# openai/multiagent-particle-envs

Measured on AMD Instinct MI355X. Metric: env steps/sec (whole node), simple_spread N=3, batch=65536 per GPU, higher is better.
Workload: dtype f32; 1 GPU; simple_spread A=3 L=3, 65536 worlds/GPU, fresh one-hot moves, reset every 25 steps; steps commanded to the step server; protocol=fresh, step-server (one doorbell per episode), batch_per_gpu=65536, global_batch=65536, mode=step-server, commands=auto, barrier_backend=none

## Files before the change

multiagent_particle_envs_amd/csrc/mpe_split.hip:

```cpp
#include <type_traits>

#include "mpe_internal.h"

#ifndef MPE_SPLIT_ABLATE
#define MPE_SPLIT_ABLATE 0
#endif

#ifdef MPE_PHASE_CLOCK
#define MPE_STAMP(k)                                                                                              \
  do {                                                                                                            \
    if (blockIdx.x < 4 && lane == 0 && b.force && t < 32)                                                         \
      reinterpret_cast<unsigned long long *>(b.force)[(((size_t)blockIdx.x * 16 + role) * 32 + t) * 8 + (k)] =     \
          __builtin_amdgcn_s_memtime();                                                                           \
  } while (0)
#else
#define MPE_STAMP(k) do { } while (0)
#endif

#ifdef MPE_DEVICE_SPAN
#define MPE_SPAN_BEGIN() const unsigned long long span_t0_ = (unsigned long long)wall_clock64()
#define MPE_SPAN_END()                                                                                             \
  do {                                                                                                             \
    if (b_in.force && (threadIdx.x & 63) == 0 && (threadIdx.x >> 6) < 8) {                                           \
      const uintptr_t sp_ = reinterpret_cast<uintptr_t>(b_in.force);                                                \
// ... 302 lines not shown
    for (int g = 0; g < NG; ++g)
#pragma unroll
      for (int v = 0; v < NADV; ++v) {
        const float d2 = sq2d(px[NADV + g] - px[v], py[NADV + g] - py[v]);
        hit[g][v] = sqrt_lt(d2, sz[NADV + g] + sz[v]);
        dmin[v] = fminf(dmin[v], d2);
      }
    float fx[2], fy[2];
#pragma unroll
    for (int f = 0; f < 2; ++f) {
      fx[f] = ROLL ? food_roll[2 * f] : (b.pos + wave_off((size_t)(2 * (A + 1 + f)) * B + w0))[ln];
      fy[f] = ROLL ? food_roll[2 * f + 1] : (b.pos + wave_off((size_t)(2 * (A + 1 + f) + 1) * B + w0))[ln];
    }
    if (live) {
#pragma unroll
      for (int a = 0; a < A; ++a) {
        float r = 0.f;
        if (a < NADV) {
          r = r - 0.1f * fast_sqrt(dmin[a < NADV ? a : 0]);
          if ((d.collide >> a) & 1u) {
#pragma unroll
            for (int g = 0; g < NG; ++g)
#pragma unroll
              for (int v = 0; v < NADV; ++v) r = r + (hit[g][v] ? 5.f : 0.f);
          }
        } else {
          if ((d.collide >> a) & 1u) {
#pragma unroll
            for (int v = 0; v < NADV; ++v) r = r - (hit[a >= NADV ? a - NADV : 0][v] ? 5.f : 0.f);
          }
          r = r - 2.f * tag_bound(fabsf(px[a]));
          r = r - 2.f * tag_bound(fabsf(py[a]));
          float m2 = INFINITY;
#pragma unroll
          for (int f = 0; f < 2; ++f) {
            const float d2 = sq2d(px[a] - fx[f], py[a] - fy[f]);
            r = r + (sqrt_lt(d2, sz[a] + sz[A + 1 + f]) ? 2.f : 0.f);
            m2 = fminf(m2, d2);
          }
          r = r + 0.05f * fast_sqrt(m2);
        }
        const size_t o = ro + (size_t)a * B;
        if (b.rew) store_aux<AUX>(b.rew + wave_off(o) + ln, r);
        if (b.done) store_aux<AUX>(b.done + wave_off(o) + ln, 0);
        if (b.info_collisions) {
          int c = 0;
          if (a < NADV) {
#pragma unroll
            for (int g = 0; g < NG; ++g) c += hit[g][a < NADV ? a : 0] ? 1 : 0;
          }
          store_aux<AUX>(b.info_collisions + wave_off(o) + ln, c);
        }
      }
    }
  }
}

typedef float vf2 __attribute__((ext_vector_type(2)));
typedef __attribute__((address_space(4))) const vf2 cvf2;
__device__ __forceinline__ vf2 pol_act2(vf2 x, bool tnh) { return vf2{pol_act(x.x, tnh), pol_act(x.y, tnh)}; }
template <int NO2>
__device__ __forceinline__ void pol_layer0(const cvf2 *W, const float *row, int sw, int D, float *rec, vf2 (&h)[NO2]) {
#pragma unroll
  for (int j = 0; j < NO2; ++j) h[j] = W[D * NO2 + j];
  for (int k = 0; k < D; ++k) {
    const float x = row[(((k >> 2) ^ sw) << 2) | (k & 3)];
    if (rec) rec[k] = x;
    const vf2 xx = {x, x};
#pragma unroll
    for (int j = 0; j < NO2; ++j) h[j] = __builtin_elementwise_fma(W[k * NO2 + j], xx, h[j]);
  }
}
template <int NO2>
__device__ __forceinline__ void pol_layer(const cvf2 *W, const vf2 (&h)[32], vf2 (&o)[NO2]) {
#pragma unroll
  for (int j = 0; j < NO2; ++j) o[j] = W[64 * NO2 + j];
#pragma unroll
  for (int k = 0; k < 64; ++k) {
    const float x = (k & 1) ? h[k >> 1].y : h[k >> 1].x;
    const vf2 xx = {x, x};
#pragma unroll
    for (int j = 0; j < NO2; ++j) o[j] = __builtin_elementwise_fma(W[k * NO2 + j], xx, o[j]);
    if ((k & 3) == 3) __builtin_amdgcn_sched_barrier(0);
  }
}
__device__ __forceinline__ void pol_logits(const float *Wg, int nl, bool tnh, const float *row, int sw, int D, float *rec,
                                           float (&z)[5]) {
  const cvf2 *W = (const cvf2 *)(uintptr_t)Wg;
  vf2 o[4];
  if (nl == 1) {
    pol_layer0<4>(W, row, sw, D, rec, o);
  } else {
    vf2 h[32];
    pol_layer0<32>(W, row, sw, D, rec, h);
#pragma unroll
    for (int j = 0; j < 32; ++j) h[j] = pol_act2(h[j], tnh);
    const cvf2 *W1 = W + (size_t)(D + 1) * 32;
    if (nl == 2) {
      pol_layer<4>(W1, h, o);
    } else {
      const cvf2 *W2 = W1 + 65 * 32;
#pragma unroll
      for (int j = 0; j < 4; ++j) o[j] = W2[64 * 4 + j];
#pragma unroll 1
      for (int c = 0; c < 4; ++c) {
        vf2 g[8];
#pragma unroll
        for (int j = 0; j < 8; ++j) g[j] = W1[64 * 32 + 8 * c + j];
#pragma unroll
        for (int k = 0; k < 64; ++k) {
          const float x = (k & 1) ? h[k >> 1].y : h[k >> 1].x;
          const vf2 xx = {x, x};
#pragma unroll
          for (int j = 0; j < 8; ++j) g[j] = __builtin_elementwise_fma(W1[k * 32 + 8 * c + j], xx, g[j]);
          if ((k & 7) == 7) __builtin_amdgcn_sched_barrier(0);
        }
#pragma unroll
        for (int u = 0; u < 16; ++u) {
          const float x = pol_act((u & 1) ? g[u >> 1].y : g[u >> 1].x, tnh);
          const vf2 xx = {x, x};
#pragma unroll
          for (int j = 0; j < 4; ++j) o[j] = __builtin_elementwise_fma(W2[(16 * c + u) * 4 + j], xx, o[j]);
        }
      }
    }
  }
  z[0] = o[0].x; z[1] = o[0].y; z[2] = o[1].x; z[3] = o[1].y; z[4] = o[2].x;
}

template <int AUX>
__device__ __forceinline__ void store_state(const MpeBuffers &b, size_t B, int i, size_t w0, unsigned ln, float mx,
                                            float my, float mvx, float mvy) {
  store_aux<AUX>(b.pos + wave_off((size_t)(2 * i) * B + w0) + ln, mx);
  store_aux<AUX>(b.pos + wave_off((size_t)(2 * i + 1) * B + w0) + ln, my);
  store_aux<AUX>(b.vel + wave_off((size_t)(2 * i) * B + w0) + ln, mvx);
  store_aux<AUX>(b.vel + wave_off((size_t)(2 * i + 1) * B + w0) + ln, mvy);
}

struct ServeArgs {
  unsigned long long *door;
  unsigned long long *flag;
  unsigned int *status;
  const float *act_ring;
  const float *comm_ring;
  int32_t ring, slots;
  unsigned long long timeout_ticks;
};
__device__ __forceinline__ unsigned long long door_load(const unsigned long long *p) {
  const unsigned long long v = __hip_atomic_load(p, __ATOMIC_RELAXED, __HIP_MEMORY_SCOPE_SYSTEM);
  const uint32_t lo = __builtin_amdgcn_readfirstlane((uint32_t)v), hi = __builtin_amdgcn_readfirstlane((uint32_t)(v >> 32));
  return ((unsigned long long)hi << 32) | lo;
}
__device__ __forceinline__ void drain_stores() { asm volatile("s_waitcnt vmcnt(0)" ::: "memory"); }

template <int KIND, int A, int L, int NADV, bool ROLL, int RP ,
          bool DUALP = false ,
          bool SERVE = false ,
          bool POL = false >
__device__ __forceinline__ void split_body(float *const g_pos, float *const g_vel, const float *const g_act, const int32_t *const g_ids,
                                           const size_t B, const int g_wpw, const int g_observe_only, const unsigned g_movable,
                                           const NarrowDesc &d, const MpeBuffers &b_in, const RollArgs &ra, const ServeArgs &sv,
                                           const PolArgs &pol) {
  static_assert(!SERVE || (ROLL && RP == kRowsSc1), "the step server: a rollout instantiation, write-through stores");
  static_assert(!POL || (ROLL && !SERVE && !DUALP), "the policy rollout: a single-role rollout instantiation");
  static_assert(!POL || KIND == MPE_SCN_SIMPLE || KIND == MPE_SCN_SPREAD || KIND == MPE_SCN_ADVERSARY || KIND == MPE_SCN_PUSH,
                "the policy rollout: scenarios whose observation rows read no other agent's velocity");
  constexpr int WM = SERVE ? kWordRowSys : (ROLL ? kWordDrawn : kWordRow);
  using S = SplitShape<KIND, A, L, NADV>;
  MPE_SPAN_BEGIN();
  MpeBuffers b = b_in;
  b.pos = g_pos;
  b.vel = g_vel;
  b.act = g_act;
  b.ids = g_ids;
  constexpr int E = A + L, XW = S::XW;
  constexpr int AUX = SERVE ? kRowsSc1 : aux_policy<KIND, RP>();
  extern __shared__ __attribute__((aligned(16))) float smem[];
  const int lane = threadIdx.x & (kWave - 1);
  constexpr bool DUAL = DUALP && ROLL;
  constexpr bool OWN_DRAW = DUAL && dual_own_draw<KIND>();
  constexpr int NAW = DUAL ? 2 * A : A;
  const int role = __builtin_amdgcn_readfirstlane((int)(threadIdx.x >> 6));
  const bool is_agent = role < NAW;
  const bool is_rows = DUAL && role >= A && role < NAW;
  const int i = is_agent ? (role >= A ? role - A : role) : 0;
  const int wpw = g_wpw;
  const size_t w0 = (size_t)blockIdx.x * (size_t)wpw;
  if (w0 >= B) return;
#ifdef MPE_STRESS_DELAY_WAVE
  if (role == (MPE_STRESS_DELAY_WAVE) % A)
    for (int k = 0; k < 10; ++k) __builtin_amdgcn_s_sleep(127);
#endif
  const int nvalid = (B - w0) < (size_t)wpw ? (int)(B - w0) : wpw;
  const bool live = lane < nvalid;
  const unsigned ln = (unsigned)(live ? lane : nvalid - 1) & 63u;
  const size_t w = w0 + (size_t)ln;
  float *const xch = smem;
  float *const tile = smem + (ROLL ? 2 : 1) * A * XW * kWave + i * S::tile_floats(ROLL);
  int *const mv = reinterpret_cast<int *>(smem + (ROLL ? 2 : 1) * A * XW * kWave + A * S::tile_floats(ROLL));

  const int T = ROLL ? ra.T : 1;
  const size_t obs_stride = (ra.trajectory || SERVE) ? (size_t)d.obs_off[A] * B : 0;
  const size_t row_stride = (ra.trajectory || SERVE) ? (size_t)A * B : 0;
  int blk0 = 0, mvt0 = 0;
  unsigned long long seen = 0;
  int *const idle_cnt = reinterpret_cast<int *>(smem + SplitShape<KIND, A, L, NADV>::lds_bytes(true) / sizeof(float));
  if constexpr (SERVE) {
    blk0 = (int)(ra.step0 % (uint64_t)sv.slots);
    mvt0 = (int)(ra.step0 % (uint64_t)sv.ring);
    if (threadIdx.x < 3) idle_cnt[threadIdx.x] = 0;
    __syncthreads();
  }
  auto block_of = [&](const int t) { return SERVE ? (blk0 + t) % sv.slots : t; };
  auto with_words = [&](const int t) {
    MpeBuffers q = b;
    if constexpr (SERVE)
      q.comm = sv.comm_ring ? sv.comm_ring + (size_t)((mvt0 + t) % sv.ring) * ((size_t)A * B * SplitShape<KIND, A, L, NADV>::DC) : nullptr;
    return q;
  };
  auto wait_door = [&](const int t, const bool publisher) -> bool {
    if constexpr (!SERVE) return true;
    const unsigned long long g = ra.step0 + (unsigned long long)t;
    if (seen > g) return true;
    seen = door_load(sv.door);
    if (seen > g) return true;
    drain_stores();
    bool told = t == 0;
    if (!publisher && !told && lane == 0) __hip_atomic_fetch_add(&idle_cnt[t & 1], 1, __ATOMIC_RELEASE, __HIP_MEMORY_SCOPE_WORKGROUP);
    const unsigned long long t_begin = (unsigned long long)wall_clock64();
    for (;;) {
      if (publisher && !told) {
        const int n = __builtin_amdgcn_readfirstlane(__hip_atomic_load(&idle_cnt[t & 1], __ATOMIC_ACQUIRE, __HIP_MEMORY_SCOPE_WORKGROUP));
        if (n >= NAW) {
          if (lane == 0) __hip_atomic_store(sv.flag + blockIdx.x, g, __ATOMIC_RELAXED, __HIP_MEMORY_SCOPE_SYSTEM);
          told = true;
        }
      }
      __builtin_amdgcn_s_sleep(4);
      seen = door_load(sv.door);
      if (seen > g) return true;
      if ((unsigned long long)wall_clock64() - t_begin > sv.timeout_ticks) {
        if (lane == 0) {
          __hip_atomic_store(sv.status, 1u, __ATOMIC_RELAXED, __HIP_MEMORY_SCOPE_SYSTEM);
          __hip_atomic_store(&idle_cnt[2], 1, __ATOMIC_RELAXED, __HIP_MEMORY_SCOPE_WORKGROUP);
        }
        return false;
      }
    }
  };
  auto next_commanded = [&](const int t) -> bool {
    if constexpr (!SERVE) return false;
    return t + 1 < T && seen > ra.step0 + (unsigned long long)t + 1;
  };
  auto aborted = [&]() -> bool {
    if constexpr (!SERVE) return false;
    return __builtin_amdgcn_readfirstlane(__hip_atomic_load(&idle_cnt[2], __ATOMIC_RELAXED, __HIP_MEMORY_SCOPE_WORKGROUP)) != 0;
  };

  if (!is_agent) {
    constexpr bool TRACK = ROLL && (KIND == MPE_SCN_CRYPTO || KIND == MPE_SCN_WORLD_COMM);
    const uint64_t gw_r = ra.world_offset + w;
    int goal_r = (ROLL && KIND == MPE_SCN_CRYPTO) ? (b.choice + wave_off(w0))[ln] : 0;
    float food[4] = {0.f, 0.f, 0.f, 0.f};
    if (ROLL && KIND == MPE_SCN_WORLD_COMM) {
#pragma unroll
      for (int f = 0; f < 2; ++f) {
        food[2 * f] = (b.pos + wave_off((size_t)(2 * (A + 1 + f)) * B + w0))[ln];
        food[2 * f + 1] = (b.pos + wave_off((size_t)(2 * (A + 1 + f) + 1) * B + w0))[ln];
      }
    }
    float sz[E];
#pragma unroll
    for (int e = 0; e < E; ++e) sz[e] = d.size[e];
    pin_s(sz);
    int cd = -1;
    uint64_t ep_r = 0;
    if (TRACK && ra.episode_len > 0) {
      const uint64_t len = (uint64_t)ra.episode_len, r = ra.step0 % len;
      cd = r == 0 ? 0 : (int)(len - r);
      ep_r = ra.step0 / len + (r ? 1 : 0);
    }
    for (int t = 0; t < T; ++t) {
      MPE_STAMP(0);
      if (SERVE && !wait_door(t, true)) {
        __syncthreads();
        return;
      }
      if (TRACK && cd >= 0) {
        if (cd == 0) {
          if (KIND == MPE_SCN_CRYPTO) goal_r = choice_draw(ra.seed, gw_r, ep_r, 0, d.choice_pop[0]);
          if (KIND == MPE_SCN_WORLD_COMM) {
#pragma unroll
            for (int f = 0; f < 2; ++f) reset_draw(ra.seed, gw_r, ep_r, A + 1 + f, ra.landmark_range, food[2 * f], food[2 * f + 1]);
          }
          ++ep_r;
          cd = ra.episode_len - 1;
        } else {
          --cd;
        }
      }
      if (ROLL && !SERVE && !OWN_DRAW && !POL && t + 1 < T) {
        const uint64_t gt1 = ra.step0 + (uint64_t)t + 1;
#pragma unroll
        for (int q = 0; q < (A + 3) / 4; ++q) {
          const U4 o = action_block(ra.seed, gw_r, gt1, q);
          const uint32_t word[4] = {o.x, o.y, o.z, o.w};
#pragma unroll
          for (int k = 0; k < 4; ++k)
            if (4 * q + k < A) mv[(((t + 1) & 1) * A + 4 * q + k) * kWave + lane] = move_of(word[k]);
        }
      }
      const float *const X = xch + (ROLL ? (t & 1) * A * XW * kWave : 0);
      MPE_STAMP(1);
      if (SERVE) drain_stores();
      __syncthreads();
      if (SERVE) {
        if (t > 0 && lane == 0) __hip_atomic_store(sv.flag + blockIdx.x, ra.step0 + (unsigned long long)t, __ATOMIC_RELAXED, __HIP_MEMORY_SCOPE_SYSTEM);
        if (lane == 0) idle_cnt[t & 1] = 0;
        if (aborted()) return;
      }
      MPE_STAMP(2);
      if (!(MPE_SPLIT_ABLATE & 2))
      reward_wave<KIND, A, L, NADV, ROLL, AUX, WM>(d, sz, with_words(t), X, lane, live, ln, B, w0, (size_t)block_of(t) * row_stride + w0,
                                                   ra.seed, gw_r, ra.step0 + (uint64_t)t, goal_r, food);
      MPE_STAMP(3);
    }
    if (SERVE) {
      drain_stores();
      __syncthreads();
      if (lane == 0) __hip_atomic_store(sv.flag + blockIdx.x, ra.step0 + (unsigned long long)T, __ATOMIC_RELAXED, __HIP_MEMORY_SCOPE_SYSTEM);
    }
    MPE_SPAN_END();
    return;
  }

  float px[E], py[E];
#pragma unroll
  for (int e = 0; e < E; ++e) {
    px[e] = (b.pos + wave_off((size_t)(2 * e) * B + w0))[ln];
    py[e] = (b.pos + wave_off((size_t)(2 * e + 1) * B + w0))[ln];
  }
  float mvx = (b.vel + wave_off((size_t)(2 * i) * B + w0))[ln];
  float mvy = (b.vel + wave_off((size_t)(2 * i + 1) * B + w0))[ln];
  const bool movable_i = (g_movable >> i) & 1u;
  const bool step_world = ROLL || !g_observe_only;
  float ux0 = 0.f, uy0 = 0.f;
  if (!ROLL && step_world && movable_i && (b.act || b.ids)) fetch_action_wave(b, B, i, w0, ln, 1.0f, ux0, uy0);

  float kc[9 + E];
  kc[0] = d.size[i]; kc[1] = d.inv_mass[i]; kc[2] = d.accel[i]; kc[3] = d.max_speed[i];
  kc[4] = d.dt; kc[5] = d.damp; kc[6] = d.cforce; kc[7] = d.cmargin; kc[8] = d.cmargin_inv;
#pragma unroll
  for (int e = 0; e < E; ++e) kc[9 + e] = d.size[e];
  pin_s(kc);
  const float size_i = kc[0], mass_i = kc[1], accel_i = kc[2], maxspd_i = kc[3];
  const float k_dt = kc[4], k_damp = kc[5], k_cforce = kc[6], k_cmargin = kc[7], k_cmargin_inv = kc[8];
  const float *const size_e = kc + 9;
  const int obs_off_i = d.obs_off[i];
  const bool collide_i = (d.collide >> i) & 1u;
  float mx = 0.f, my = 0.f;
#pragma unroll
  for (int a = 0; a < A; ++a)
    if (a == i) { mx = px[a]; my = py[a]; }

  const uint64_t gw = ra.world_offset + w;
  constexpr bool HAS_GOAL = KIND == MPE_SCN_ADVERSARY || KIND == MPE_SCN_PUSH;
  constexpr int NCH = S::NCH, DC = S::DC;
  int goal = NCH >= 1 ? (b.choice + wave_off(w0))[ln] : 0;
  int pick1 = NCH >= 2 ? (b.choice + wave_off(B + w0))[ln] : 0;

  int countdown = -1;
  uint64_t ep = 0;
  if (ROLL && ra.episode_len > 0) {
    const uint64_t len = (uint64_t)ra.episode_len, r = ra.step0 % len;
    countdown = r == 0 ? 0 : (int)(len - r);
    ep = ra.step0 / len + (r ? 1 : 0);
  }

  float gx = 0.f, gy = 0.f;
  [[maybe_unused]] bool did_reset = false;
  auto roll_reset = [&]() -> bool {
    const bool reset_now = countdown == 0;
    if (countdown >= 0) countdown = reset_now ? ra.episode_len - 1 : countdown - 1;
    if (reset_now) {
#pragma unroll
      for (int e = 0; e < E; ++e) reset_draw(ra.seed, gw, ep, e, e < A ? 1.0f : ra.landmark_range, px[e], py[e]);
#pragma unroll
      for (int a = 0; a < A; ++a)
        if (a == i) { mx = px[a]; my = py[a]; }
      mvx = 0.f;
      mvy = 0.f;
      if (NCH >= 1) goal = choice_draw(ra.seed, gw, ep, 0, d.choice_pop[0]);
      if (NCH >= 2) pick1 = choice_draw(ra.seed, gw, ep, 1, d.choice_pop[1]);
      ++ep;
      if (SERVE) did_reset = true;
    }
    return reset_now;
  };
  [[maybe_unused]] float pa1 = 0.f, pa2 = 0.f, pa3 = 0.f, pa4 = 0.f;
  auto step_forces = [&](const int t, float &fx, float &fy) {
    float ux, uy;
    const uint64_t gt = ra.step0 + (uint64_t)t;
    if (ROLL) {
      if constexpr (!POL) roll_reset();
      if constexpr (SERVE) {
        const float *const mt = sv.act_ring + (size_t)((mvt0 + t) % sv.ring) * ((size_t)A * B * MPE_ACTION_DIM);
        typedef float vf4 __attribute__((ext_vector_type(4)));
        const float *const mp = mt + wave_off(((size_t)i * B + w0) * MPE_ACTION_DIM) + (ln * MPE_ACTION_DIM + 1);
        vf4 m4;
        asm volatile("global_load_dwordx4 %0, %1, off sc0 sc1\n\ts_waitcnt vmcnt(0)" : "=&v"(m4) : "v"(mp) : "memory");
        if (movable_i) {
          ux = (m4.x - m4.y) * accel_i;
          uy = (m4.z - m4.w) * accel_i;
        } else {
          ux = 0.f;
          uy = 0.f;
        }
      } else if constexpr (POL) {
        ux = (pa1 - pa2) * accel_i;
        uy = (pa3 - pa4) * accel_i;
      } else {
      const int m = (t == 0 || OWN_DRAW) ? action_draw(ra.seed, gw, gt, i) : mv[((t & 1) * A + i) * kWave + lane];
      ux = ((m == 1 ? 1.f : 0.f) - (m == 2 ? 1.f : 0.f)) * accel_i;
      uy = ((m == 3 ? 1.f : 0.f) - (m == 4 ? 1.f : 0.f)) * accel_i;
      }
    } else if (step_world && movable_i) {
      if (b.act || b.ids) { ux = ux0 * accel_i; uy = uy0 * accel_i; }
      else fetch_action_wave(b, B, i, w0, ln, accel_i, ux, uy);
    } else {
      ux = 0.f;
      uy = 0.f;
    }
    fx = ux + 0.f;
    fy = uy + 0.f;
    if (movable_i && step_world && collide_i && !(MPE_SPLIT_ABLATE & 1)) {
#pragma unroll
      for (int j = 0; j < E; ++j) {
        if (j == i) continue;
        if (!((d.collide >> j) & 1u)) continue;
        float cx, cy;
        contact_force(mx - px[j], my - py[j], size_i + size_e[j], k_cforce, k_cmargin, k_cmargin_inv, cx, cy);
        fx = cx + fx;
        fy = cy + fy;
      }
    }
  };
  auto step_integrate = [&](const int t, const float fx, const float fy) {
    if (movable_i && step_world) {
      integrate_one(mx, my, mvx, mvy, fx, fy, mass_i, maxspd_i, k_damp, k_dt);
#ifdef MPE_STRESS_STORE_BEFORE_BARRIER
      if (live && (!ROLL || t == T - 1)) store_state<AUX>(b, B, i, w0, ln, mx, my, mvx, mvy);
#endif
    }
#ifdef MPE_PHASE_CLOCK
    asm volatile("" ::"v"(mx), "v"(my), "v"(mvx), "v"(mvy));
#endif
  };
  auto publish = [&](const int t) {
    float *const X = xch + (ROLL ? (t & 1) * A * XW * kWave : 0);
    X[(i * XW + 0) * kWave + lane] = mx;
    X[(i * XW + 1) * kWave + lane] = my;
    X[(i * XW + 2) * kWave + lane] = mvx;
    X[(i * XW + 3) * kWave + lane] = mvy;
    if (KIND == MPE_SCN_SPREAD) {
#pragma unroll
      for (int l = 0; l < L; ++l) X[(i * XW + 4 + l) * kWave + lane] = sq2d(mx - px[A + l], my - py[A + l]);
    }
    if (KIND == MPE_SCN_SIMPLE) X[(i * XW + 4) * kWave + lane] = sq2d(mx - px[A], my - py[A]);
    if (HAS_GOAL || KIND == MPE_SCN_SPEAKER_LISTENER) {
      goal_pos<A, L>(px, py, goal, gx, gy);
      X[(i * XW + 4) * kWave + lane] = sq2d(mx - gx, my - gy);
    }
    if constexpr (KIND == MPE_SCN_REFERENCE) {
      goal_pos<A, L>(px, py, i == 0 ? pick1 : goal, gx, gy);
      X[(i * XW + 4) * kWave + lane] = sq2d(mx - gx, my - gy);
    }
    if constexpr (KIND == MPE_SCN_WORLD_COMM) {
#pragma unroll
      for (int f = 0; f < 2; ++f)
        X[(i * XW + 4 + f) * kWave + lane] =
            sqrt_lt(sq2d(mx - px[A + 3 + f], my - py[A + 3 + f]), size_i + size_e[A + 3 + f]) ? 1.f : -1.f;
    }
  };
  auto behind_barrier = [&](const int t) {
#ifndef MPE_STRESS_STORE_BEFORE_BARRIER
    if (movable_i && step_world && live && (!ROLL || (SERVE ? !next_commanded(t) : t == T - 1)) && !(MPE_SPLIT_ABLATE & 8))
      store_state<AUX>(b, B, i, w0, ln, mx, my, mvx, mvy);
#endif
    if constexpr (SERVE) {
      if (did_reset && live) {
#pragma unroll
        for (int l = 0; l < L; ++l)
          if (l % A == i) {
            store_aux<AUX>(b.pos + wave_off((size_t)(2 * (A + l)) * B + w0) + ln, px[A + l]);
            store_aux<AUX>(b.pos + wave_off((size_t)(2 * (A + l) + 1) * B + w0) + ln, py[A + l]);
          }
        if (NCH >= 1 && i == 0) {
          store_aux<AUX>(b.choice + wave_off(w0) + ln, goal);
          if (NCH >= 2) store_aux<AUX>(b.choice + wave_off(B + w0) + ln, pick1);
        }
        if (!movable_i) store_state<AUX>(b, B, i, w0, ln, mx, my, mvx, mvy);
      }
      did_reset = false;
    }
    if constexpr (KIND == MPE_SCN_ADVERSARY && !ROLL) {
      if (live && b.info_rew) {
        store_aux<AUX>(b.info_rew + wave_off((size_t)i * B + w0) + ln, sq2d(mx - gx, my - gy));
        if (b.info_min_dists) {
#pragma unroll
          for (int l = 0; l < L; ++l)
            store_aux<AUX>(b.info_min_dists + wave_off(((size_t)l * A + i) * B + w0) + ln, sq2d(mx - px[A + l], my - py[A + l]));
        }
      }
    }
    const float *const X = xch + (ROLL ? (t & 1) * A * XW * kWave : 0);
#pragma unroll
    for (int a = 0; a < A; ++a) {
      if (a == i) { px[a] = mx; py[a] = my; continue; }
      px[a] = X[(a * XW + 0) * kWave + lane];
      py[a] = X[(a * XW + 1) * kWave + lane];
    }
#ifdef MPE_PHASE_CLOCK
#pragma unroll
    for (int a = 0; a < A; ++a) asm volatile("" ::"v"(px[a]), "v"(py[a]));
#endif
  };
  [[maybe_unused]] int pol_D = 0, pol_S = 0, pol_sw = 0;
  auto note_tile = [&](auto dc, auto pc) {
    if constexpr (POL) {
      constexpr int D = decltype(dc)::value;
      constexpr bool P = decltype(pc)::value;
      constexpr int NS = (P && row_vec4<D>()) ? D / 4 : 0;
      pol_D = D;
      pol_S = P ? pair_stride<D>() : tile_stride<D>();
      pol_sw = NS ? swz4<NS>(lane) : 0;
    }
  };
  auto rows = [&](const int t, const bool pre) {
    if (MPE_SPLIT_ABLATE & 4) return;
    const float *const X = xch + (ROLL ? (t & 1) * A * XW * kWave : 0);
    const uint64_t gt = ra.step0 + (uint64_t)t;
    float *const obs_t = b.obs + (size_t)block_of(t) * obs_stride;
    [[maybe_unused]] const MpeBuffers bw = with_words(t);
    if (KIND == MPE_SCN_SIMPLE) {
      constexpr int D = 2 + 2 * L;
      {
        RowPairs<D> r(tile, lane);
        r.put(0, mvx, mvy);
#pragma unroll
        for (int l = 0; l < L; ++l) r.put(2 + 2 * l, px[A + l] - mx, py[A + l] - my);
      }
      note_tile(std::integral_constant<int, D>{}, std::bool_constant<true>{});
        if (!pre) flush_rows<D, true, RP>(tile, obs_t + B * obs_off_i + w0 * D, nvalid, lane, d.vec4);
    }
    if (KIND == MPE_SCN_SPREAD) {
      constexpr int D = 4 + 2 * L + 4 * (A - 1);
      {
        RowPairs<D> r(tile, lane);
        r.put(0, mvx, mvy);
        r.put(2, mx, my);
#pragma unroll
        for (int l = 0; l < L; ++l) r.put(4 + 2 * l, px[A + l] - mx, py[A + l] - my);
        int k = 4 + 2 * L;
#pragma unroll
        for (int j = 0; j < A; ++j) {
          if (j == i) continue;
// ... 128 lines not shown
      constexpr int D = 2 + 2 * L + 3 + DC, RS = tile_stride<D>();
      const int mine = i == 0 ? goal : pick1;
      put1<RS>(tile, lane, 0, mvx); put1<RS>(tile, lane, 1, mvy);
#pragma unroll
      for (int l = 0; l < L; ++l) { put1<RS>(tile, lane, 2 + 2 * l, px[A + l] - mx); put1<RS>(tile, lane, 3 + 2 * l, py[A + l] - my); }
#pragma unroll
      for (int c = 0; c < 3; ++c) put1<RS>(tile, lane, 2 + 2 * L + c, mine == c ? 0.75f : 0.25f);
      const Word<WM> co = word_of<DC, WM>(bw, B, w0, ln, 1 - i, ra.seed, gw, gt);
#pragma unroll
      for (int c = 0; c < DC; ++c) put1<RS>(tile, lane, 5 + 2 * L + c, co[c]);
      note_tile(std::integral_constant<int, D>{}, std::bool_constant<false>{});
        if (!pre) flush_rows<D, false, RP>(tile, obs_t + B * obs_off_i + w0 * D, nvalid, lane, d.vec4);
    }
    if constexpr (KIND == MPE_SCN_CRYPTO) {
      const Word<WM> cs = word_of<DC, WM>(bw, B, w0, ln, 2, ra.seed, gw, gt);
      static_assert((DC & 1) == 0, "crypto rows are written as pairs");
      if (i == 0) {
        constexpr int D = DC;
        RowPairs<D> r(tile, lane);
#pragma unroll
        for (int c = 0; c < DC; c += 2) r.put(c, cs[c], cs[c + 1]);
        note_tile(std::integral_constant<int, D>{}, std::bool_constant<true>{});
        if (!pre) flush_rows<D, true, RP>(tile, obs_t + B * obs_off_i + w0 * D, nvalid, lane, d.vec4);
      } else {
        constexpr int D = 2 * DC;
        RowPairs<D> r(tile, lane);
        const int first = i == 1 ? pick1 : goal;
#pragma unroll
        for (int c = 0; c < DC; c += 2) r.put(c, first == c ? 1.f : 0.f, first == c + 1 ? 1.f : 0.f);
#pragma unroll
        for (int c = 0; c < DC; c += 2) {
          if (i == 1) r.put(DC + c, cs[c], cs[c + 1]);
          else        r.put(DC + c, pick1 == c ? 1.f : 0.f, pick1 == c + 1 ? 1.f : 0.f);
        }
        note_tile(std::integral_constant<int, D>{}, std::bool_constant<true>{});
        if (!pre) flush_rows<D, true, RP>(tile, obs_t + B * obs_off_i + w0 * D, nvalid, lane, d.vec4);
      }
    }
    if constexpr (KIND == MPE_SCN_WORLD_COMM) {
      constexpr int NG = A - NADV;
      constexpr int DA = 4 + 2 * L + 2 * (A - 1) + 2 * NG + 2 + DC, DGd = 4 + 2 * L + 2 * (A - 1) + 2 + 2 * (NG - 1);
      const bool f1 = X[(i * XW + 4) * kWave + lane] > 0.f, f2 = X[(i * XW + 5) * kWave + lane] > 0.f;
      bool vis[A];
#pragma unroll
      for (int j = 0; j < A; ++j) {
        const bool o1 = X[(j * XW + 4) * kWave + lane] > 0.f, o2 = X[(j * XW + 5) * kWave + lane] > 0.f;
        vis[j] = i == 0 || (f1 && o1) || (f2 && o2) || (!f1 && !o1 && !f2 && !o2);
      }
      auto row = [&](auto dsel, auto advt) {
        constexpr int D = decltype(dsel)::value, RS = tile_stride<D>();
        constexpr bool ADV = decltype(advt)::value;
        constexpr bool HALF = S::trows(ROLL) == 32;
#pragma unroll
        for (int h = 0; h < (HALF ? 2 : 1); ++h) {
        const int r = HALF ? (lane & 31) : lane;
        if (!HALF || (lane >> 5) == h) {
        int k = 0;
        put1<RS>(tile, r, 0, mvx); put1<RS>(tile, r, 1, mvy); put1<RS>(tile, r, 2, mx); put1<RS>(tile, r, 3, my);
        k = 4;
#pragma unroll
        for (int l = 0; l < L; ++l) { put1<RS>(tile, r, k, px[A + l] - mx); put1<RS>(tile, r, k + 1, py[A + l] - my); k += 2; }
#pragma unroll
        for (int j = 0; j < A; ++j) {
          if (j == i) continue;
          put1<RS>(tile, r, k, vis[j] ? px[j] - mx : 0.f);
          put1<RS>(tile, r, k + 1, vis[j] ? py[j] - my : 0.f);
          k += 2;
        }
        if (!ADV) { put1<RS>(tile, r, k, f1 ? 1.f : -1.f); put1<RS>(tile, r, k + 1, f2 ? 1.f : -1.f); k += 2; }
#pragma unroll
        for (int j = NADV; j < A; ++j) {
          if (j == i) continue;
          put1<RS>(tile, r, k, vis[j] ? X[(j * XW + 2) * kWave + lane] : 0.f);
          put1<RS>(tile, r, k + 1, vis[j] ? X[(j * XW + 3) * kWave + lane] : 0.f);
          k += 2;
        }
        if (ADV) {
          put1<RS>(tile, r, k, f1 ? 1.f : -1.f); put1<RS>(tile, r, k + 1, f2 ? 1.f : -1.f); k += 2;
          const Word<WM> cl = word_of<DC, WM>(bw, B, w0, ln, 0, ra.seed, gw, gt);
#pragma unroll
          for (int c = 0; c < DC; ++c) put1<RS>(tile, r, k + c, cl[c]);
        }
        }
        const int nv = HALF ? min(max(nvalid - 32 * h, 0), 32) : nvalid;
        if (nv > 0) flush_rows<D, false, RP>(tile, obs_t + B * obs_off_i + (w0 + (HALF ? 32 * h : 0)) * D, nv, lane, d.vec4);
        }
      };
      if (i < NADV) row(std::integral_constant<int, DA>{}, std::true_type{});
      else          row(std::integral_constant<int, DGd>{}, std::false_type{});
    }
  };
  [[maybe_unused]] auto decide = [&](const int t) {
    const uint64_t gt = ra.step0 + (uint64_t)t;
    const bool rs = roll_reset();
    if (t == 0 || rs) {
      if (HAS_GOAL) goal_pos<A, L>(px, py, goal, gx, gy);
      rows(t, true);
    }
    float *const rec = (pol.obs_in && live) ? pol.obs_in + wave_off((size_t)t * (size_t)d.obs_off[A] * B + B * (size_t)obs_off_i + w0 * (size_t)pol_D) +
                                                  ln * pol_D
                                            : nullptr;
    float z[5];
    pol_logits(pol.w + pol.off[i], pol.nl[i], pol.act[i] != 0, tile + lane * pol_S, pol_sw, pol_D, rec, z);
    float zm = z[0];
    int am = 0;
#pragma unroll
    for (int j = 1; j < 5; ++j)
      if (z[j] > zm) { zm = z[j]; am = j; }
    float e[5], sum = 0.f;
#pragma unroll
    for (int j = 0; j < 5; ++j) {
      e[j] = __expf(z[j] - zm);
      sum += e[j];
    }
    float r[5];
    int m = am;
    if (pol.mode == MPE_POLICY_SOFTMAX) {
#pragma unroll
      for (int j = 0; j < 5; ++j) r[j] = e[j] / sum;
    } else {
      if (pol.mode == MPE_POLICY_SAMPLE) {
        const float u = (float)(policy_bits(pol.seed, gw, gt, i) >> 8) * (1.0f / 16777216.0f);
        float c = 0.f;
        m = 4;
        float cj[4];
#pragma unroll
        for (int j = 0; j < 4; ++j) {
          c += e[j] / sum;
          cj[j] = c;
        }
#pragma unroll
        for (int j = 3; j >= 0; --j)
          if (u < cj[j]) m = j;
      }
#pragma unroll
      for (int j = 0; j < 5; ++j) r[j] = j == m ? 1.f : 0.f;
    }
    if (live) {
      float *const ar = pol.act_out + wave_off((((size_t)t * A + i) * B + w0) * MPE_ACTION_DIM) + ln * MPE_ACTION_DIM;
#pragma unroll
      for (int j = 0; j < 5; ++j) ar[j] = r[j];
      if (pol.logp) {
        float zsel = z[0];
#pragma unroll
        for (int j = 1; j < 5; ++j) zsel = m == j ? z[j] : zsel;
        (pol.logp + wave_off(((size_t)t * A + i) * B + w0))[ln] = (zsel - zm) - __logf(sum);
      }
    }
    pa1 = r[1];
    pa2 = r[2];
    pa3 = r[3];
    pa4 = r[4];
  };
  if constexpr (DUAL) {
    if (is_rows) {
      for (int t = 0; t < T; ++t) {
        MPE_STAMP(0);
        const bool reset_now = countdown == 0;
        if (countdown >= 0) countdown = reset_now ? ra.episode_len - 1 : countdown - 1;
        if (reset_now) {
#pragma unroll
          for (int l = 0; l < L; ++l) reset_draw(ra.seed, gw, ep, A + l, ra.landmark_range, px[A + l], py[A + l]);
          if (NCH >= 1) goal = choice_draw(ra.seed, gw, ep, 0, d.choice_pop[0]);
          if (NCH >= 2) pick1 = choice_draw(ra.seed, gw, ep, 1, d.choice_pop[1]);
          ++ep;
        }
        if (HAS_GOAL || KIND == MPE_SCN_SPEAKER_LISTENER) goal_pos<A, L>(px, py, goal, gx, gy);
        MPE_STAMP(2);
        __syncthreads();
        if (SERVE && aborted()) return;
        MPE_STAMP(3);
        const float *const X = xch + (t & 1) * A * XW * kWave;
        mx = X[(i * XW + 0) * kWave + lane];
        my = X[(i * XW + 1) * kWave + lane];
        mvx = X[(i * XW + 2) * kWave + lane];
        mvy = X[(i * XW + 3) * kWave + lane];
#pragma unroll
        for (int a = 0; a < A; ++a) {
          if (a == i) { px[a] = mx; py[a] = my; continue; }
          px[a] = X[(a * XW + 0) * kWave + lane];
          py[a] = X[(a * XW + 1) * kWave + lane];
        }
#ifdef MPE_PHASE_CLOCK
#pragma unroll
        for (int a = 0; a < A; ++a) asm volatile("" ::"v"(px[a]), "v"(py[a]));
#endif
        MPE_STAMP(4);
        rows(t, false);
        MPE_STAMP(5);
        if constexpr (SERVE) {
          drain_stores();
          if (lane == 0) __hip_atomic_fetch_add(&idle_cnt[(t + 1) & 1], 1, __ATOMIC_RELEASE, __HIP_MEMORY_SCOPE_WORKGROUP);
        }
      }
      if (SERVE) __syncthreads();
      MPE_SPAN_END();
      return;
    }
    float fx, fy;
    { [[maybe_unused]] const int t = 0; MPE_STAMP(0); }
    if (SERVE && !wait_door(0, false)) {
      __syncthreads();
      return;
    }
    step_forces(0, fx, fy);
    step_integrate(0, fx, fy);
    { [[maybe_unused]] const int t = 0; MPE_STAMP(1); }
    publish(0);
    for (int t = 0; t < T; ++t) {
      MPE_STAMP(2);
      if (SERVE) drain_stores();
      __syncthreads();
      if (SERVE && aborted()) return;
      MPE_STAMP(3);
      behind_barrier(t);
      MPE_STAMP(4);
      if (t + 1 < T) {
        if (SERVE && !wait_door(t + 1, false)) {
          __syncthreads();
          return;
        }
        step_forces(t + 1, fx, fy);
        step_integrate(t + 1, fx, fy);
        MPE_STAMP(5);
        publish(t + 1);
      }
    }
    if (SERVE) {
      drain_stores();
      __syncthreads();
      MPE_SPAN_END();
      return;
    }
  } else {
    for (int t = 0; t < T; ++t) {
      float fx, fy;
      MPE_STAMP(0);
      if (SERVE && !wait_door(t, false)) {
        __syncthreads();
        return;
      }
      if constexpr (POL) decide(t);
      step_forces(t, fx, fy);
      step_integrate(t, fx, fy);
      MPE_STAMP(1);
      publish(t);
      MPE_STAMP(2);
      if (SERVE) drain_stores();
      __syncthreads();
      if (SERVE && aborted()) return;
      MPE_STAMP(3);
      behind_barrier(t);
      MPE_STAMP(4);
      rows(t, false);
      MPE_STAMP(5);
    }
    if (SERVE) {
      drain_stores();
      __syncthreads();
      MPE_SPAN_END();
      return;
    }
  }
  if (ROLL && NCH >= 1 && ra.episode_len > 0 && live && i == 0) {
    store_aux<AUX>(b.choice + wave_off(w0) + ln, goal);
    if (NCH >= 2) store_aux<AUX>(b.choice + wave_off(B + w0) + ln, pick1);
  }
  if (ROLL && ((speakers_of<KIND>() >> i) & 1u) && live && T > 0) {
    float *const mine = const_cast<float *>(b.comm) + wave_off(((size_t)i * B + w0) * DC) + ln * DC;
    const int id = comm_draw(ra.seed, gw, ra.step0 + (uint64_t)(T - 1), i, DC);
#pragma unroll
    for (int c = 0; c < DC; ++c) mine[c] = c == id ? 1.f : 0.f;
  }
  if (ROLL && ra.episode_len > 0 && live) {
#pragma unroll
    for (int l = 0; l < L; ++l)
      if (l % A == i) {
        (b.pos + wave_off((size_t)(2 * (A + l)) * B + w0))[ln] = px[A + l];
        (b.pos + wave_off((size_t)(2 * (A + l) + 1) * B + w0))[ln] = py[A + l];
      }
    if (!movable_i) {
      store_aux<AUX>(b.pos + wave_off((size_t)(2 * i) * B + w0) + ln, mx);
      store_aux<AUX>(b.pos + wave_off((size_t)(2 * i + 1) * B + w0) + ln, my);
      store_aux<AUX>(b.vel + wave_off((size_t)(2 * i) * B + w0) + ln, mvx);
      store_aux<AUX>(b.vel + wave_off((size_t)(2 * i + 1) * B + w0) + ln, mvy);
    }
  }
  MPE_SPAN_END();
}

template <int KIND, int A, int L, int NADV, bool ROLL, int RP, bool DUALP = false, bool SERVE = false>
__global__ void __launch_bounds__((SplitShape<KIND, A, L, NADV>::waves(DUALP) * kWave))
k_split(float *const g_pos, float *const g_vel, const float *const g_act, const int32_t *const g_ids, const size_t B,
        const int g_wpw, const int g_observe_only, const unsigned g_movable, const NarrowDesc d, const MpeBuffers b_in,
        const RollArgs ra, const ServeArgs sv) {
  split_body<KIND, A, L, NADV, ROLL, RP, DUALP, SERVE, false>(g_pos, g_vel, g_act, g_ids, B, g_wpw, g_observe_only, g_movable, d, b_in,
                                                              ra, sv, PolArgs{});
}
template <int KIND, int A, int L, int NADV>
__global__ void __launch_bounds__((SplitShape<KIND, A, L, NADV>::waves(false) * kWave))
k_split_policy(float *const g_pos, float *const g_vel, const float *const g_act, const int32_t *const g_ids, const size_t B,
               const int g_wpw, const int g_observe_only, const unsigned g_movable, const NarrowDesc d, const MpeBuffers b_in,
               const RollArgs ra, const PolArgs pol) {
  split_body<KIND, A, L, NADV, true, kRowsNt, false, false, true>(g_pos, g_vel, g_act, g_ids, B, g_wpw, g_observe_only, g_movable, d,
                                                                  b_in, ra, ServeArgs{}, pol);
}


constexpr size_t kRowsNtFromBytes = 8u << 20, kRollNtFromBytes = 12u << 20;
using SplitFn = void (*)(float *, float *, const float *, const int32_t *, const size_t, const int, const int, const unsigned,
                         const NarrowDesc, const MpeBuffers, const RollArgs, const ServeArgs);
struct SplitEntry {
  int kind, A, L, nadv;
  SplitFn step, step_small, roll, roll_small;
  SplitFn roll_dual, roll_dual_small;
  SplitFn serve, serve_dual;
  size_t lds_step, lds_roll;
};
template <int KIND, int A, int L, int NADV>
constexpr SplitFn serve_fn() { return k_split<KIND, A, L, NADV, true, kRowsSc1, false, true>; }
template <int KIND, int A, int L, int NADV>
constexpr SplitFn serve_dual_fn() {
  if constexpr (dual_kind<KIND>() && SplitShape<KIND, A, L, NADV>::waves(true) * kWave <= 1024)
    return k_split<KIND, A, L, NADV, true, kRowsSc1, true, true>;
  else return nullptr;
}
template <int KIND, int A, int L, int NADV, int RP>
constexpr SplitFn dual_fn() {
  if constexpr (dual_kind<KIND>() && SplitShape<KIND, A, L, NADV>::waves(true) * kWave <= 1024) return k_split<KIND, A, L, NADV, true, RP, true>;
  else return nullptr;
}
#define MPE_SPLIT_ENTRY(KIND, A, L, NADV)                                                                         \
  { KIND, A, L, NADV, k_split<KIND, A, L, NADV, false, kRowsNt>, k_split<KIND, A, L, NADV, false, kRowsSc1>,       \
    k_split<KIND, A, L, NADV, true, kRowsNt>, k_split<KIND, A, L, NADV, true, kRowsSc1>,                           \
    dual_fn<KIND, A, L, NADV, kRowsNt>(), dual_fn<KIND, A, L, NADV, kRowsSc1>(), serve_fn<KIND, A, L, NADV>(),     \
    serve_dual_fn<KIND, A, L, NADV>(),                                                                             \
    SplitShape<KIND, A, L, NADV>::lds_bytes(false), SplitShape<KIND, A, L, NADV>::lds_bytes(true) }

static const SplitEntry kSplitTable[] = {
    MPE_SPLIT_ENTRY(MPE_SCN_SIMPLE, 1, 1, 0),
    MPE_SPLIT_ENTRY(MPE_SCN_SPREAD, 1, 1, 0), MPE_SPLIT_ENTRY(MPE_SCN_SPREAD, 2, 2, 0),
    MPE_SPLIT_ENTRY(MPE_SCN_SPREAD, 3, 3, 0), MPE_SPLIT_ENTRY(MPE_SCN_SPREAD, 4, 4, 0),
    MPE_SPLIT_ENTRY(MPE_SCN_SPREAD, 5, 5, 0), MPE_SPLIT_ENTRY(MPE_SCN_SPREAD, 6, 6, 0),
    MPE_SPLIT_ENTRY(MPE_SCN_TAG, 4, 2, 3), MPE_SPLIT_ENTRY(MPE_SCN_TAG, 2, 1, 1),
    MPE_SPLIT_ENTRY(MPE_SCN_TAG, 6, 3, 4),
    MPE_SPLIT_ENTRY(MPE_SCN_ADVERSARY, 3, 2, 1), MPE_SPLIT_ENTRY(MPE_SCN_PUSH, 2, 2, 1),
    MPE_SPLIT_ENTRY(MPE_SCN_SPEAKER_LISTENER, 2, 3, 0), MPE_SPLIT_ENTRY(MPE_SCN_REFERENCE, 2, 3, 0),
    MPE_SPLIT_ENTRY(MPE_SCN_CRYPTO, 3, 2, 1), MPE_SPLIT_ENTRY(MPE_SCN_WORLD_COMM, 6, 5, 4),
#ifdef MPE_SPLIT_TEAM_GRID
    MPE_SPLIT_ENTRY(MPE_SCN_ADVERSARY, 2, 1, 1), MPE_SPLIT_ENTRY(MPE_SCN_ADVERSARY, 3, 2, 2),
    MPE_SPLIT_ENTRY(MPE_SCN_ADVERSARY, 4, 3, 1), MPE_SPLIT_ENTRY(MPE_SCN_ADVERSARY, 4, 3, 2),
    MPE_SPLIT_ENTRY(MPE_SCN_ADVERSARY, 5, 4, 1), MPE_SPLIT_ENTRY(MPE_SCN_ADVERSARY, 5, 4, 2),
    MPE_SPLIT_ENTRY(MPE_SCN_ADVERSARY, 6, 5, 1), MPE_SPLIT_ENTRY(MPE_SCN_ADVERSARY, 6, 5, 2),
    MPE_SPLIT_ENTRY(MPE_SCN_WORLD_COMM, 3, 5, 2), MPE_SPLIT_ENTRY(MPE_SCN_WORLD_COMM, 4, 5, 3),
    MPE_SPLIT_ENTRY(MPE_SCN_WORLD_COMM, 5, 5, 4), MPE_SPLIT_ENTRY(MPE_SCN_WORLD_COMM, 6, 5, 5),
    MPE_SPLIT_ENTRY(MPE_SCN_WORLD_COMM, 4, 5, 2), MPE_SPLIT_ENTRY(MPE_SCN_WORLD_COMM, 5, 5, 3),
    MPE_SPLIT_ENTRY(MPE_SCN_WORLD_COMM, 7, 5, 5),
    MPE_SPLIT_ENTRY(MPE_SCN_WORLD_COMM, 5, 5, 2), MPE_SPLIT_ENTRY(MPE_SCN_WORLD_COMM, 6, 5, 3),
    MPE_SPLIT_ENTRY(MPE_SCN_WORLD_COMM, 7, 5, 4), MPE_SPLIT_ENTRY(MPE_SCN_WORLD_COMM, 8, 5, 5),
#endif
};

static const SplitEntry *find_split(int kind, int A, int L, int nadv) {
  for (const SplitEntry &e : kSplitTable)
    if (e.kind == kind && e.A == A && e.L == L && (kind < MPE_SCN_TAG || e.nadv == nadv)) return &e;
  return nullptr;
}

bool split_supports(int kind, int A, int L, int nadv) { return find_split(kind, A, L, nadv) != nullptr; }

int launch_split(bool roll, int kind, int A, int L, int nadv, const NarrowDesc &d, const MpeBuffers &b, size_t B,
                 const RollArgs &ra, hipStream_t stream) {
  const SplitEntry *e = find_split(kind, A, L, nadv);
  if (!e) return MPE_EUNSUPPORTED;
  RollArgs r2 = ra;
#ifdef MPE_SPLIT_WPW
  r2.wpw = MPE_SPLIT_WPW;
#else
  r2.wpw = kWave;
#endif
  const unsigned grid = (unsigned)((B + r2.wpw - 1) / r2.wpw);
  const size_t row_bytes = (size_t)d.obs_off[A] * sizeof(float) * B;
  const bool small = row_bytes < (roll ? kRollNtFromBytes : kRowsNtFromBytes);
  SplitFn fn = roll ? (small ? e->roll_small : e->roll) : small ? e->step_small : e->step;
  int waves = A + 1;
  static const int n_cu = [] {
    int dev = 0, v = 0;
    if (hipGetDevice(&dev) == hipSuccess && hipDeviceGetAttribute(&v, hipDeviceAttributeMultiprocessorCount, dev) == hipSuccess && v > 0) return v;
    (void)hipGetLastError();
    return 256;
  }();
#ifdef MPE_SPLIT_DUAL_MAX_WG_PER_CU_X2
  const unsigned dual_max = (unsigned)n_cu * (MPE_SPLIT_DUAL_MAX_WG_PER_CU_X2) / 2;
#else
  const unsigned dual_max = (unsigned)n_cu * 3 / 2;
#endif
  SplitFn dual = small ? e->roll_dual_small : e->roll_dual;
  if (roll && dual && grid <= dual_max) {
    fn = dual;
    waves = 2 * A + 1;
  }
  hipLaunchKernelGGL(fn, dim3(grid), dim3(waves * kWave), roll ? e->lds_roll : e->lds_step, stream,
                     b.pos, b.vel, b.act, b.ids, B, (int)r2.wpw, (int)r2.observe_only, (unsigned)d.movable, d, b, r2, ServeArgs{});
  return (int)hipGetLastError();
// ... 114 lines not shown
```

Before: 19.16 billion env-steps/s.

## Prefetch next step's move into AGPRs and defer store drains in step server

In the step-server path, agent waves now issue the next step's action-ring load into accumulation registers (a0-a3) once the doorbell already covers that step. The load then overlaps the row/observation work and is consumed later with a counted s_waitcnt, which removes a blocking load-and-wait from each step's critical path. The store drain before the per-step barrier moves to after it, on the publisher side. Abort paths gain explicit drain-plus-sync and step-count publishing. The counted vmcnt and the hand-written AGPR usage depend on exact store counts and register allocation, so wrong counts or compiler clobbering could give silent data hazards.

```diff
diff --git a/multiagent_particle_envs_amd/csrc/mpe_split.hip b/multiagent_particle_envs_amd/csrc/mpe_split.hip
--- a/multiagent_particle_envs_amd/csrc/mpe_split.hip
+++ b/multiagent_particle_envs_amd/csrc/mpe_split.hip
@@ -478,6 +478,16 @@
   return ((unsigned long long)hi << 32) | lo;
 }
 __device__ __forceinline__ void drain_stores() { asm volatile("s_waitcnt vmcnt(0)" ::: "memory"); }
+
+template <int KIND, int A, int L, int NADV>
+constexpr int serve_row_stores() {
+  int D = 0;
+  if (KIND == MPE_SCN_SIMPLE) D = 2 + 2 * L;
+  if (KIND == MPE_SCN_SPREAD) D = 4 + 2 * L + 4 * (A - 1);
+  if (D == 0) return 0;
+  const bool aligned = (D % 4) == 0 ? (((D / 4) & 1) == 1 || D == 8 || D == 16 || D == 32) : ((D % 2) == 0 && ((D / 2) % 2) == 1);
+  return aligned ? (16 * D + kWave - 1) / kWave : 0;
+}
 
 template <int KIND, int A, int L, int NADV, bool ROLL, int RP ,
           bool DUALP = false ,
@@ -530,6 +540,7 @@
   const size_t row_stride = (ra.trajectory || SERVE) ? (size_t)A * B : 0;
   int blk0 = 0, mvt0 = 0;
   unsigned long long seen = 0;
+  [[maybe_unused]] unsigned long long pub = ra.step0;
   int *const idle_cnt = reinterpret_cast<int *>(smem + SplitShape<KIND, A, L, NADV>::lds_bytes(true) / sizeof(float));
   if constexpr (SERVE) {
     blk0 = (int)(ra.step0 % (uint64_t)sv.slots);
@@ -559,6 +570,7 @@
         const int n = __builtin_amdgcn_readfirstlane(__hip_atomic_load(&idle_cnt[t & 1], __ATOMIC_ACQUIRE, __HIP_MEMORY_SCOPE_WORKGROUP));
         if (n >= NAW) {
           if (lane == 0) __hip_atomic_store(sv.flag + blockIdx.x, g, __ATOMIC_RELAXED, __HIP_MEMORY_SCOPE_SYSTEM);
+          pub = g;
           told = true;
         }
       }
@@ -582,6 +594,19 @@
     if constexpr (!SERVE) return false;
     return __builtin_amdgcn_readfirstlane(__hip_atomic_load(&idle_cnt[2], __ATOMIC_RELAXED, __HIP_MEMORY_SCOPE_WORKGROUP)) != 0;
   };
+  auto leave_aborted = [&]() {
+    drain_stores();
+    __syncthreads();
+  };
+  auto publish_steps = [&](const int n) {
+    if constexpr (SERVE) {
+      const unsigned long long c = ra.step0 + (unsigned long long)(n > 0 ? n : 0);
+      if (c > pub) {
+        if (lane == 0) __hip_atomic_store(sv.flag + blockIdx.x, c, __ATOMIC_RELAXED, __HIP_MEMORY_SCOPE_SYSTEM);
+        pub = c;
+      }
+    }
+  };
 
   if (!is_agent) {
     constexpr bool TRACK = ROLL && (KIND == MPE_SCN_CRYPTO || KIND == MPE_SCN_WORLD_COMM);
@@ -610,6 +635,8 @@
       MPE_STAMP(0);
       if (SERVE && !wait_door(t, true)) {
         __syncthreads();
+        leave_aborted();
+        publish_steps(t);
         return;
       }
       if (TRACK && cd >= 0) {
@@ -638,12 +665,16 @@
       }
       const float *const X = xch + (ROLL ? (t & 1) * A * XW * kWave : 0);
       MPE_STAMP(1);
-      if (SERVE) drain_stores();
       __syncthreads();
       if (SERVE) {
-        if (t > 0 && lane == 0) __hip_atomic_store(sv.flag + blockIdx.x, ra.step0 + (unsigned long long)t, __ATOMIC_RELAXED, __HIP_MEMORY_SCOPE_SYSTEM);
+        drain_stores();
+        publish_steps(t - (DUAL ? 0 : 1));
         if (lane == 0) idle_cnt[t & 1] = 0;
-        if (aborted()) return;
+        if (aborted()) {
+          leave_aborted();
+          publish_steps(t);
+          return;
+        }
       }
       MPE_STAMP(2);
       if (!(MPE_SPLIT_ABLATE & 2))
@@ -724,20 +755,52 @@
     return reset_now;
   };
   [[maybe_unused]] float pa1 = 0.f, pa2 = 0.f, pa3 = 0.f, pa4 = 0.f;
+  constexpr bool PREFETCH = SERVE && A + L <= 8 &&
+                            (KIND == MPE_SCN_SIMPLE || KIND == MPE_SCN_SPREAD || KIND == MPE_SCN_SPEAKER_LISTENER ||
+                             KIND == MPE_SCN_REFERENCE || (KIND == MPE_SCN_TAG && A == 2));
+  [[maybe_unused]] bool have_pf = false;
+  [[maybe_unused]] auto move_ptr = [&](const int t) -> const float * {
+    const float *const mt = sv.act_ring + (size_t)((mvt0 + t) % sv.ring) * ((size_t)A * B * MPE_ACTION_DIM);
+    return mt + wave_off(((size_t)i * B + w0) * MPE_ACTION_DIM) + (ln * MPE_ACTION_DIM + 1);
+  };
+  [[maybe_unused]] auto prefetch_move = [&](const int t) {
+    if constexpr (PREFETCH) {
+      if (next_commanded(t)) {
+        const float *const mp = move_ptr(t + 1);
+        asm volatile("global_load_dwordx4 a[0:3], %0, off sc0 sc1" : : "v"(mp) : "memory", "a0", "a1", "a2", "a3");
+        have_pf = true;
+      }
+    }
+  };
+  constexpr int NROW = (PREFETCH && !DUAL) ? serve_row_stores<KIND, A, L, NADV>() : 0;
+  const bool rows_counted = NROW > 0 && nvalid == kWave && d.vec4;
   auto step_forces = [&](const int t, float &fx, float &fy) {
     float ux, uy;
     const uint64_t gt = ra.step0 + (uint64_t)t;
     if (ROLL) {
       if constexpr (!POL) roll_reset();
       if constexpr (SERVE) {
-        const float *const mt = sv.act_ring + (size_t)((mvt0 + t) % sv.ring) * ((size_t)A * B * MPE_ACTION_DIM);
         typedef float vf4 __attribute__((ext_vector_type(4)));
-        const float *const mp = mt + wave_off(((size_t)i * B + w0) * MPE_ACTION_DIM) + (ln * MPE_ACTION_DIM + 1);
-        vf4 m4;
-        asm volatile("global_load_dwordx4 %0, %1, off sc0 sc1\n\ts_waitcnt vmcnt(0)" : "=&v"(m4) : "v"(mp) : "memory");
+        float m1, m2, m3, m4;
+        if (PREFETCH && have_pf) {
+#define MPE_TAKE_MOVE(CNT)                                                                                                       \
+  asm volatile("s_waitcnt vmcnt(%4)\n\tv_accvgpr_read_b32 %0, a0\n\tv_accvgpr_read_b32 %1, a1\n\tv_accvgpr_read_b32 %2, a2\n\t" \
+               "v_accvgpr_read_b32 %3, a3"                                                                                      \
+               : "=v"(m1), "=v"(m2), "=v"(m3), "=v"(m4) : "n"(CNT) : "memory", "a0", "a1", "a2", "a3")
+          if (rows_counted) MPE_TAKE_MOVE(NROW);
+          else MPE_TAKE_MOVE(0);
+#undef MPE_TAKE_MOVE
+          have_pf = false;
+        } else {
+          const float *const mp = move_ptr(t);
+          vf4 mq;
+          asm volatile("global_load_dwordx4 %0, %1, off sc0 sc1\n\ts_waitcnt vmcnt(0)" : "=&v"(mq) : "v"(mp) : "memory");
+          m1 = mq.x; m2 = mq.y; m3 = mq.z; m4 = mq.w;
+        }
+        if constexpr (DUAL) prefetch_move(t);
         if (movable_i) {
-          ux = (m4.x - m4.y) * accel_i;
-          uy = (m4.z - m4.w) * accel_i;
+          ux = (m1 - m2) * accel_i;
+          uy = (m3 - m4) * accel_i;
         } else {
           ux = 0.f;
           uy = 0.f;
@@ -1172,6 +1235,11 @@
     pa3 = r[3];
     pa4 = r[4];
   };
+  if constexpr (SERVE) {
+#pragma unroll
+    for (int e = 0; e < E; ++e) asm volatile("" ::"v"(px[e]), "v"(py[e]));
+    asm volatile("" ::"v"(mvx), "v"(mvy), "v"(goal), "v"(pick1));
+  }
   if constexpr (DUAL) {
     if (is_rows) {
       for (int t = 0; t < T; ++t) {
@@ -1188,7 +1256,10 @@
         if (HAS_GOAL || KIND == MPE_SCN_SPEAKER_LISTENER) goal_pos<A, L>(px, py, goal, gx, gy);
         MPE_STAMP(2);
         __syncthreads();
-        if (SERVE && aborted()) return;
+        if (SERVE && aborted()) {
+          leave_aborted();
+          return;
+        }
         MPE_STAMP(3);
         const float *const X = xch + (t & 1) * A * XW * kWave;
         mx = X[(i * XW + 0) * kWave + lane];
@@ -1221,6 +1292,7 @@
     { [[maybe_unused]] const int t = 0; MPE_STAMP(0); }
     if (SERVE && !wait_door(0, false)) {
       __syncthreads();
+      leave_aborted();
       return;
     }
     step_forces(0, fx, fy);
@@ -1229,15 +1301,18 @@
     publish(0);
     for (int t = 0; t < T; ++t) {
       MPE_STAMP(2);
-      if (SERVE) drain_stores();
       __syncthreads();
-      if (SERVE && aborted()) return;
+      if (SERVE && aborted()) {
+        leave_aborted();
+        return;
+      }
       MPE_STAMP(3);
       behind_barrier(t);
       MPE_STAMP(4);
       if (t + 1 < T) {
         if (SERVE && !wait_door(t + 1, false)) {
           __syncthreads();
+          leave_aborted();
           return;
         }
         step_forces(t + 1, fx, fy);
@@ -1258,6 +1333,7 @@
       MPE_STAMP(0);
       if (SERVE && !wait_door(t, false)) {
         __syncthreads();
+        leave_aborted();
         return;
       }
       if constexpr (POL) decide(t);
@@ -1266,10 +1342,13 @@
       MPE_STAMP(1);
       publish(t);
       MPE_STAMP(2);
-      if (SERVE) drain_stores();
       __syncthreads();
-      if (SERVE && aborted()) return;
+      if (SERVE && aborted()) {
+        leave_aborted();
+        return;
+      }
       MPE_STAMP(3);
+      if constexpr (SERVE) prefetch_move(t);
       behind_barrier(t);
       MPE_STAMP(4);
       rows(t, false);
```

Result: slower. 18.78 billion env-steps/s (-1.9%).
